# keichi/sdn-mpi-router

Hardware: AMD Instinct MI355X
Metric: all-pairs routes/sec + % HBM roofline, k=48 fat-tree, 1/2/4/8 MI355X (higher is better)
Workload: dtype int32; 1 GPU; fat_tree:48 all-pairs dfs route tables (find_route); fabric=fat_tree:48, V=2880, E=110592, table_layout=packed, endpoints=host-bearing switches (host pairs), parallelism=sources sharded over 1 GPU(s), steps_in_flight=1

## Files before the change

### sdn-mpi-router_amd/csrc/capi.hip

```cpp
#include <stdarg.h>
#include <stdio.h>
#include <stdlib.h>
#include <string.h>

#include <algorithm>
#include <array>
#include <map>
#include <string>
#include <thread>
#include <vector>

#include "common.h"

static thread_local char g_err[512] = "";

int sdnr_fail(int code, const char *fmt, ...)
{
    va_list ap;
    va_start(ap, fmt);
    vsnprintf(g_err, sizeof g_err, fmt, ap);
    va_end(ap);
    return code;
}

// ... 130 lines not shown
}

static void free_graph(sdnr_ctx *c)
{
    int32_t **bufs[] = {&c->row_ptr, &c->col, &c->port, &c->ell_col, &c->ell_port};
    for (int32_t **b : bufs) {
        if (*b) (void)hipFree(*b);
        *b = nullptr;
    }
    if (c->cost) (void)hipFree(c->cost);
    c->cost = nullptr;
    c->has_cost = false;
    if (c->twin_rep) (void)hipFree(c->twin_rep);
    c->twin_rep = nullptr;
    c->has_twins = false;
    ++c->upload_gen;
    memset(c->live_ring, 0, sizeof c->live_ring);
    if (c->radj16 && c->radj_owned) (void)hipFree(c->radj16);
    if (c->runs) (void)hipFree(c->runs);
    c->runs = nullptr;
    c->runs_R = 0;
    if (c->adjb) (void)hipFree(c->adjb);
    if (c->adjp) (void)hipFree(c->adjp);
    if (c->radjx) (void)hipFree(c->radjx);
    c->adjb = nullptr;
    c->adjp = nullptr;
    c->radjx = nullptr;
    if (c->q_radj16 && c->q_radj_owned) (void)hipFree(c->q_radj16);
    {
        void **qb[] = {reinterpret_cast<void **>(&c->q_adj16), reinterpret_cast<void **>(&c->q_deg32),
                       reinterpret_cast<void **>(&c->q_radjw), reinterpret_cast<void **>(&c->q_radjc),
                       reinterpret_cast<void **>(&c->q_cid), reinterpret_cast<void **>(&c->q_info),
                       reinterpret_cast<void **>(&c->q_loff), reinterpret_cast<void **>(&c->q_slot),
                       reinterpret_cast<void **>(&c->q_tab)};
        for (void **b : qb) {
            if (*b) (void)hipFree(*b);
            *b = nullptr;
        }
    }
    c->q_radj16 = nullptr;
    c->q_radj_owned = false;
    c->q_V = c->q_E = 0;
    if (c->adj16) (void)hipFree(c->adj16);
    if (c->deg32) (void)hipFree(c->deg32);
    if (c->radjw) (void)hipFree(c->radjw);
    c->radjw = nullptr;
    if (c->radjc) (void)hipFree(c->radjc);
    c->radjc = nullptr;
    if (c->dict_bp) (void)hipFree(c->dict_bp);
    if (c->dict_bt) (void)hipFree(c->dict_bt);
    if (c->dict_off) (void)hipFree(c->dict_off);
    c->dict_bp = nullptr;
    c->dict_bt = nullptr;
    c->dict_off = nullptr;
    c->dict_P = 0;
    c->dict_NB = 0;
    c->dict_bpw = 0;
    if (c->ell16) (void)hipFree(c->ell16);
    if (c->ell_hi) (void)hipFree(c->ell_hi);
    c->ell16 = nullptr;
    c->ell_hi = nullptr;
    c->adj16 = nullptr;
    c->radj16 = nullptr;
    c->deg32 = nullptr;
    c->radj_owned = false;
    c->radj_pair = false;
    c->V = -1;
// ... 591 lines not shown
            if (he == hipSuccess) he = hipMalloc(reinterpret_cast<void **>(&ctx->adjp), ap.size());
            if (he == hipSuccess)
                he = hipMemcpyAsync(ctx->adjp, ap.data(), ap.size(), hipMemcpyHostToDevice,
                                    ctx->stream);
            if (he == hipSuccess) he = hipMalloc(reinterpret_cast<void **>(&ctx->radjx), rx.size() * 4);
            if (he == hipSuccess)
                he = hipMemcpyAsync(ctx->radjx, rx.data(), rx.size() * 4, hipMemcpyHostToDevice,
                                    ctx->stream);
            if (he == hipSuccess) he = hipStreamSynchronize(ctx->stream);
        }
#endif
        if (he == hipSuccess) he = hipStreamSynchronize(ctx->stream);
        if (he != hipSuccess) {
            free_graph(ctx);
            return sdnr_hip_fail(he, "graph_upload(adj16)");
        }
        if (ctx->has_twins && ctx->radj16) {
            std::vector<int32_t> cmax_of((size_t)V), id_of((size_t)V, -1);
            for (int32_t v = 0; v < V; ++v) cmax_of[twin_rep[v]] = v;
            int32_t Vq = 0;
            for (int32_t v = 0; v < V; ++v)
                if (cmax_of[twin_rep[v]] == v) id_of[twin_rep[v]] = Vq++;
            std::vector<uint32_t> cidrk((size_t)V + kPad, 0u), info((size_t)Vq + 1, 0u),
                csize((size_t)Vq, 0u);
            for (int32_t v = 0; v < V; ++v) {
                const uint32_t c = (uint32_t)id_of[twin_rep[v]];
                cidrk[v] = c | (csize[c]++ << 16);
                info[c] = (uint32_t)v;
            }
            for (int32_t c = 0; c < Vq; ++c) info[c] |= csize[c] > 1 ? 1u << 16 : 0u;
            std::vector<int32_t> qptr((size_t)Vq + 1, 0), qcol, tmp;
            std::vector<uint32_t> loff((size_t)Vq * SDNR_WAVE + kPad, 0u);
            std::vector<uint8_t> mslot;
            for (int32_t c = 0; c < Vq; ++c) {
                const int32_t P = (int32_t)(info[c] & 0xFFFFu);
                tmp.clear();
                for (int32_t e = row_ptr[P]; e < row_ptr[P + 1]; ++e)
                    tmp.push_back((int32_t)(cidrk[col[e]] & 0xFFFFu));
                std::sort(tmp.begin(), tmp.end());
                tmp.erase(std::unique(tmp.begin(), tmp.end()), tmp.end());
                for (size_t j = 0; j < tmp.size(); ++j) {
                    loff[(size_t)c * SDNR_WAVE + j] = (uint32_t)mslot.size();
                    mslot.resize(mslot.size() + csize[tmp[j]], 0);
                }
                for (int32_t e = row_ptr[P]; e < row_ptr[P + 1]; ++e) {
                    const uint32_t ck = cidrk[col[e]];
                    const size_t j = (size_t)(std::lower_bound(tmp.begin(), tmp.end(),
                                                               (int32_t)(ck & 0xFFFFu)) - tmp.begin());
                    mslot[loff[(size_t)c * SDNR_WAVE + j] + (ck >> 16)] = (uint8_t)(e - row_ptr[P]);
                }
                qcol.insert(qcol.end(), tmp.begin(), tmp.end());
                qptr[(size_t)c + 1] = (int32_t)qcol.size();
            }
            mslot.resize(mslot.size() + kPad, 0);
            qcol.push_back(0);
            std::vector<uint16_t> qa16, qr16;
            bool qsym = true;
            int32_t qmaxin = 0;
            U16Rows q;
            he = upload_u16_rows(q, Vq, qptr.data(), qcol.data(), qa16, qr16, qsym, qmaxin,
                                 ctx->radj_pair ? 1 : 0);
            ctx->q_adj16 = q.adj16;
            ctx->q_radj16 = q.radj16;
            ctx->q_deg32 = q.deg32;
            ctx->q_radjw = q.radjw;
            ctx->q_radjc = q.radjc;
            ctx->q_radj_owned = q.radj_owned;
            auto put = [&](void **dst, const void *src, size_t bytes) {
                if (he == hipSuccess) he = hipMalloc(dst, bytes);
                if (he == hipSuccess)
                    he = hipMemcpyAsync(*dst, src, bytes, hipMemcpyHostToDevice, ctx->stream);
            };
            put(reinterpret_cast<void **>(&ctx->q_cid), cidrk.data(), cidrk.size() * 4);
            put(reinterpret_cast<void **>(&ctx->q_info), info.data(), info.size() * 4);
            put(reinterpret_cast<void **>(&ctx->q_loff), loff.data(), loff.size() * 4);
            put(reinterpret_cast<void **>(&ctx->q_slot), mslot.data(), mslot.size());
            const sdnr_quot qt{V, ctx->q_cid, ctx->q_info, ctx->q_loff, ctx->q_slot};
            put(reinterpret_cast<void **>(&ctx->q_tab), &qt, sizeof qt);
            if (he == hipSuccess) he = hipStreamSynchronize(ctx->stream);
            if (he != hipSuccess) {
                free_graph(ctx);
                return sdnr_hip_fail(he, "graph_upload(quotient)");
            }
            if (!ctx->radjw && ctx->q_radjw) {
                (void)hipFree(ctx->q_radjw);
                ctx->q_radjw = nullptr;
            }
            if (!ctx->radjc && ctx->q_radjc) {
                (void)hipFree(ctx->q_radjc);
                ctx->q_radjc = nullptr;
            }
            ctx->q_V = Vq;
            ctx->q_E = qptr[(size_t)Vq];
        }
    }
    bool symmetric = true;
    for (int32_t u = 0; u < V && symmetric; ++u)
        for (int32_t e = row_ptr[u]; e < row_ptr[u + 1]; ++e) {
            const int32_t v = col[e];
            int32_t lo = row_ptr[v], hi = row_ptr[v + 1];
            while (lo < hi) {
                const int32_t mid = (lo + hi) >> 1;
                if (col[mid] < u) lo = mid + 1; else hi = mid;
            }
            if (lo == row_ptr[v + 1] || col[lo] != u) {
                symmetric = false;
                break;
            }
        }
    SDNR_HIP(hipStreamSynchronize(ctx->stream));
// ... 1069 lines not shown
```

### sdn-mpi-router_amd/csrc/common.h

```cpp
#pragma once

#include <hip/hip_runtime.h>
#include <stdlib.h>
#include <stdint.h>
#include <stddef.h>

#include "../../include/sdnroute.h"

#define SDNR_WAVE 64
#define SDNR_LDS_PER_CU (160 * 1024)
#define SDNR_MAX_LDS_PER_BLOCK (160 * 1024)


__device__ __forceinline__ int lane_id() { return (int)__lane_id(); }

__device__ __forceinline__ int lanes_below(uint64_t m) {
    return (int)__builtin_amdgcn_mbcnt_hi((uint32_t)(m >> 32),
                                          __builtin_amdgcn_mbcnt_lo((uint32_t)m, 0u));
}

__device__ __forceinline__ int uniform(int x) {
    return __builtin_amdgcn_readfirstlane(x);
}

__device__ __forceinline__ int read_lane(int x, int lane) {
    return __builtin_amdgcn_readlane(x, lane);
}

__device__ __forceinline__ int highest_lane(uint64_t m) { return 63 - __clzll(m); }

__device__ __forceinline__ int lds_swz(int x) { return x ^ ((x >> 3) & 31); }


constexpr int kLiveRing = 8;

struct sdnr_quot {
    int32_t VR;
    const uint32_t *cid, *info, *loff;
    const uint8_t *slot;
};

struct sdnr_ctx {
    int device = 0;
    int num_cus = 256;
    hipStream_t own_stream = nullptr;
    hipStream_t stream = nullptr;

    int32_t V = -1, E = 0, max_deg = 0;
    uint64_t deg2_sum = 0;
    int32_t max_indeg = 0x7FFFFFFF;
    int32_t W = 0;
    int32_t *row_ptr = nullptr, *col = nullptr, *port = nullptr;
    uint32_t *cost = nullptr;
    bool has_cost = false;
    int32_t *ell_col = nullptr, *ell_port = nullptr;
    uint16_t *ell16 = nullptr;
    uint32_t *ell_hi = nullptr;
    uint32_t *dict_bp = nullptr;
    uint32_t *dict_bt = nullptr;
    int32_t *dict_off = nullptr;
    int32_t dict_P = 0, dict_NB = 0, dict_bpw = 0;
    uint16_t *adj16 = nullptr;
    uint16_t *radj16 = nullptr;
    uint32_t *deg32 = nullptr;
    uint16_t *radjw = nullptr;
    uint16_t *radjc = nullptr;
    bool radj_owned = false;
    bool radj_pair = false;
    uint32_t *runs = nullptr;
    int32_t runs_R = 0;
    uint64_t *adjb = nullptr;
    uint8_t *adjp = nullptr;
    uint32_t *radjx = nullptr;
    int32_t *twin_rep = nullptr;
    bool has_twins = false;
    int32_t q_V = 0, q_E = 0;
    uint16_t *q_adj16 = nullptr, *q_radj16 = nullptr, *q_radjw = nullptr, *q_radjc = nullptr;
    uint32_t *q_deg32 = nullptr;
    bool q_radj_owned = false;
    uint32_t *q_cid = nullptr, *q_info = nullptr, *q_loff = nullptr;
    uint8_t *q_slot = nullptr;
    struct sdnr_quot *q_tab = nullptr;
    bool dfs_quotient = false;
    int32_t dfs_nsrc = 0;
    bool dfs_folded = false;
    int32_t dfs_form = 0;
    unsigned long long *h_live = nullptr;
    struct {
        uint32_t seq0, seq1, gen;
        int32_t nsrc;
    } live_ring[kLiveRing] = {};
    int live_head = 0;
    uint32_t live_seq = 0;
    uint32_t upload_gen = 0;

    void *scratch = nullptr;
    size_t scratch_bytes = 0;
    void *stage = nullptr;
    size_t stage_bytes = 0;
    void *scratch2 = nullptr;
    size_t scratch2_bytes = 0;
    void *scratch3 = nullptr;
    size_t scratch3_bytes = 0;
    void *wq = nullptr;
    size_t wq_bytes = 0;
    void *dmat = nullptr;
    size_t dmat_bytes = 0;
    void *anc = nullptr;
    size_t anc_bytes = 0;
    const void *anc_parent = nullptr, *anc_port = nullptr;
    size_t anc_n = 0;
    bool anc_valid = false;
    bool port16 = false;
    bool symmetric = false;
// ... 190 lines not shown
```

### sdn-mpi-router_amd/csrc/dfs.hip

```cpp
#include <stdlib.h>
#include <string.h>

#include <type_traits>

#include "common.h"

namespace {

constexpr int kRing = 1024;

template <bool ELL, bool HOPS>
__global__ __launch_bounds__(64) void dfs_lds_wide_kernel(
    int V, int W, const int32_t *__restrict__ row_ptr,
    const int32_t *__restrict__ col, const int32_t *__restrict__ port,
    const int32_t *__restrict__ src, int nsrc, int32_t *__restrict__ out_parent,
    int32_t *__restrict__ out_port, int32_t *__restrict__ out_hops)
{
    extern __shared__ __attribute__((aligned(16))) uint32_t lds[];
    const int VW = (V + 31) >> 5;
    const int VWp = (VW + 3) & ~3;
    uint32_t *vis = lds;
    uint32_t *stk = vis + VWp;
    uint32_t *ps = stk + V;
    uint16_t *dep = reinterpret_cast<uint16_t *>(ps + V);
// ... 1402 lines not shown
            for (int v = lane; v < V; v += SDNR_WAVE) {
                if (((vis[vsw(v >> 5)] >> (v & 31)) & 1u) == 0u) {
                    prow[v] = -1;
                    if (!PACKED) trow[v] = -1;
                    if (HOPS) put_hop(out_hops, hb + v, -1, flags);
                }
            }
        }
        __builtin_amdgcn_fence(__ATOMIC_RELEASE, "workgroup", "local");
        if (lane == 0) __hip_atomic_store(&ctl[2 * NS + w], -1, __ATOMIC_RELAXED,
                                          __HIP_MEMORY_SCOPE_WORKGROUP);
#ifdef SDNR_STAMPS
        SDNR_STAMP(z_t1);
        if (lane == 0) {
            atomicAdd(&g_stamp[0], z_t1 - z_t0);
            atomicAdd(&g_stamp[1], z_rd);
            atomicAdd(&g_stamp[2], z_it);
            atomicAdd(&g_stamp[3], z_nl);
            atomicAdd(&g_stamp[4], z_qw);
            atomicAdd(&g_stamp[5], z_push);
            atomicAdd(&g_stamp[6], z_sp);
            atomicAdd(&g_stamp[7], z_rf);
            atomicAdd(&g_stamp[8], z_rfc);
        }
#endif
    } else {
        split_writer<NS, HOPS, PK>(V, W, ell_port, qrec, qdep, ctl, lane, out_parent, out_port,
                                   out_hops, err, flags);
    }
}

__device__ __forceinline__ int swz(int x) { return lds_swz(x); }

template <int NW, bool HOPS, bool PACKED, bool C16, int PAIR, bool SPEC = false, bool QUOT = false>
__global__ __launch_bounds__(NW * 64, C16 ? 7 : 1) void dfs_async_kernel(
    int V, const uint16_t *__restrict__ adj, const uint16_t *__restrict__ radj,
    const uint32_t *__restrict__ deg, const int32_t *__restrict__ row_ptr,
    const int32_t *__restrict__ port, int W, const int32_t *__restrict__ ell_port,
    const int32_t *__restrict__ src, int nsrc, int32_t *__restrict__ out_parent,
    int32_t *__restrict__ out_port, int32_t *__restrict__ out_hops, int *__restrict__ err,
    int flags, const int32_t *__restrict__ live,
    const sdnr_quot *__restrict__ qt)
{
    static_assert(NW >= 2, "wave 0 searches, the others decrement");
    constexpr bool quot = QUOT;
    const int VT = quot ? uniform((int)qt->VR) : V;
    if (live) nsrc = min(nsrc, *live);
    constexpr int U = 4;
    constexpr int S = NW - 1;
    constexpr int RING = 512;
#ifndef SDNR_ASYNC_G
#define SDNR_ASYNC_G 8
#endif
#ifndef SDNR_ASYNC_FLUSH_U
#define SDNR_ASYNC_FLUSH_U 6
#endif
#ifndef SDNR_ASYNC_G_DW
#define SDNR_ASYNC_G_DW 16
#endif
#ifndef SDNR_ASYNC_G_P1
#define SDNR_ASYNC_G_P1 8
#endif
#ifndef SDNR_ASYNC_G_U16
#define SDNR_ASYNC_G_U16 48
#endif
#ifndef SDNR_ASYNC_G_DW4
#define SDNR_ASYNC_G_DW4 32
#endif
    constexpr int G = NW <= 4 ? (PAIR == 0 ? SDNR_ASYNC_G_U16
                                           : (PAIR == 2 && NW == 4 ? SDNR_ASYNC_G_DW4 : SDNR_ASYNC_G))
                              : (PAIR == 2 ? SDNR_ASYNC_G_DW : (PAIR == 1 ? SDNR_ASYNC_G_P1 : 8));
    constexpr unsigned kSpin = 1u << 22;
    extern __shared__ __attribute__((aligned(16))) uint32_t lds[];
    const int VW = (V + 1 + 31) >> 5;
    const int VWp = (VW + 3) & ~3;
    const int CWp = ((((C16 ? (V + 2) >> 1 : V + 1) + 31) & ~31) + 64 + 255) & ~255;
    const int SWp = (((V + 1) >> 1) + 3) & ~3;
    const int PW = (V + 255) & ~255;
    const int PWp = C16 ? PW / 2 + PW / 4 : PW;
    uint32_t *vis = lds;
    uint32_t *cnt = vis + VWp;
    uint16_t *stk = reinterpret_cast<uint16_t *>(cnt + CWp);
    uint32_t *ps = cnt + CWp + SWp;
    uint16_t *ps16 = reinterpret_cast<uint16_t *>(ps);
    uint8_t *sl8 = reinterpret_cast<uint8_t *>(ps16 + PW);
    uint16_t *dep = reinterpret_cast<uint16_t *>(ps + PWp);
    auto cnt_of = [&](int v) -> uint32_t {
        if constexpr (C16) {
            const uint32_t x = __hip_atomic_load(&cnt[swz(v >> 1)], __ATOMIC_RELAXED,
                                                 __HIP_MEMORY_SCOPE_WORKGROUP);
            return (x >> ((v & 1) << 4)) & 0xFFFFu;
        } else {
            return __hip_atomic_load(&cnt[swz(v)], __ATOMIC_RELAXED, __HIP_MEMORY_SCOPE_WORKGROUP);
        }
    };
    uint16_t *ring = reinterpret_cast<uint16_t *>(ps + PWp + (HOPS ? ((V + 1) >> 1) : 0));
    int *ctl = reinterpret_cast<int *>(ring + RING);
    const int lane = lane_id();
    const int w = uniform((int)(threadIdx.x >> 6));
#ifdef SDNR_STAMPS
    unsigned long long kstart;
    SDNR_STAMP(kstart);
#endif

    for (int si = blockIdx.x; si < nsrc; si += gridDim.x) {
        const int sr = uniform(src[si]);
        int32_t *prow = out_parent + (size_t)si * VT;
        int32_t *trow = PACKED ? nullptr : out_port + (size_t)si * VT;
        const size_t hb = (size_t)si * VT;
        if (sr < 0 || sr >= VT) {
            for (int v = threadIdx.x; v < VT; v += blockDim.x) {
                prow[v] = -1;
                if (!PACKED) trow[v] = -1;
                if (HOPS) put_hop(out_hops, hb + v, -1, flags);
            }
            continue;
        }
        int s = sr;
        bool rootvis = true;
        if constexpr (quot) {
            s = uniform((int)(qt->cid[sr] & 0xFFFFu));
            rootvis = uniform((int)(qt->info[s] >> 16)) == 0;
        }
#ifdef SDNR_STAMPS
        unsigned long long ph0, ph1, ph2, ph3;
        SDNR_STAMP(ph0);
#endif
        for (int i = threadIdx.x; i < VW; i += blockDim.x) vis[i] = 0u;
        if constexpr (C16) {
            const int nw = (V + 2) >> 1;
            for (int i0 = threadIdx.x; i0 < nw; i0 += U * blockDim.x) {
                uint2 dg[U];
#pragma unroll
                for (int k = 0; k < U; ++k) {
                    const int i = i0 + k * (int)blockDim.x;
                    dg[k] = reinterpret_cast<const uint2 *>(deg)[i < nw ? i : 0];
                }
#pragma unroll
                for (int k = 0; k < U; ++k) {
                    const int i = i0 + k * (int)blockDim.x;
                    if (i < nw) cnt[swz(i)] = dg[k].x | (dg[k].y << 16);
                }
            }
        } else {
            for (int i0 = threadIdx.x; i0 <= V; i0 += U * blockDim.x) {
                uint32_t dg[U];
#pragma unroll
                for (int k = 0; k < U; ++k) {
                    const int i = i0 + k * (int)blockDim.x;
                    dg[k] = deg[i <= V ? i : V];
                }
#pragma unroll
                for (int k = 0; k < U; ++k) {
                    const int i = i0 + k * (int)blockDim.x;
                    if (i <= V) cnt[swz(i)] = dg[k];
                }
            }
        }
        if (threadIdx.x < 2 + S) ctl[threadIdx.x] = 0;
        __syncthreads();
#ifdef SDNR_STAMPS
        SDNR_STAMP(ph1);
#endif

        if (w == 0) {
            if (flags & kFlagPrio) __builtin_amdgcn_s_setprio(3);
            const int pub0 = rootvis ? 1 : 0;
            if (lane == 0) {
                if (rootvis) vis[s >> 5] |= 1u << (s & 31);
                vis[V >> 5] |= 1u << (V & 31);
                if (C16) ps16[swz(s)] = (uint16_t)s;
                else ps[swz(s)] = (uint32_t)s;
                if (HOPS) dep[s] = 0;
                stk[0] = (uint16_t)s;
                ring[0] = (uint16_t)s;
            }
            __builtin_amdgcn_fence(__ATOMIC_RELEASE, "workgroup");
            if (lane == 0) __hip_atomic_store(&ctl[0], pub0, __ATOMIC_RELAXED, __HIP_MEMORY_SCOPE_WORKGROUP);
            int pub = pub0, pubd = pub0, sp = 1, lo = 0;
            constexpr int NPF = 1;
            int pu[NPF];
            uint16_t xp[NPF];
#pragma unroll
            for (int k = 0; k < NPF; ++k) {
                pu[k] = -1;
                xp[k] = (uint16_t)V;
            }
#ifdef SDNR_STAMPS
            unsigned long long st_t0, st_t1, st_row = 0, st_cand = 0, st_false = 0, st_bp = 0,
                                               st_miss = 0, st_skip = 0, st_tc = 0, st_skipc = 0,
                                               st_pushc = 0;
            SDNR_STAMP(st_t0);
// ... 127 lines not shown
                    m = __ballot(c != 0u);
                    if (m) break;
                    sp -= kk;
                }
                if (pub != pubd) {
                    __builtin_amdgcn_fence(__ATOMIC_RELEASE, "workgroup", "local");
                    if (lane == 0) __hip_atomic_store(&ctl[0], pub, __ATOMIC_RELAXED,
                                                      __HIP_MEMORY_SCOPE_WORKGROUP);
                    pubd = pub;
                }
                if (!m) break;
                const int first = __ffsll((unsigned long long)m) - 1;
                sp -= first + 1;
                for (int u = read_lane(e, first); u >= 0;) u = explore(u);
            }
            __builtin_amdgcn_fence(__ATOMIC_RELEASE, "workgroup");
            if (lane == 0) __hip_atomic_store(&ctl[1], 1, __ATOMIC_RELAXED, __HIP_MEMORY_SCOPE_WORKGROUP);
            if (flags & kFlagPrio) __builtin_amdgcn_s_setprio(0);
#ifdef SDNR_STAMPS
            SDNR_STAMP(st_t1);
            if (lane == 0) {
                atomicAdd(&g_stamp[0], st_t1 - st_t0);
                atomicAdd(&g_stamp[1], st_row);
                atomicAdd(&g_stamp[2], st_cand);
                atomicAdd(&g_stamp[3], st_false);
                atomicAdd(&g_stamp[4], st_bp);
                atomicAdd(&g_stamp[5], st_skip * 1000000ull + st_miss);
                atomicAdd(&g_stamp[6], st_skipc);
                atomicAdd(&g_stamp[7], st_pushc);
            }
#endif
        } else {
            int j = w - 1;
            for (unsigned spin = 0;;) {
                const int P = __hip_atomic_load(&ctl[0], __ATOMIC_ACQUIRE, __HIP_MEMORY_SCOPE_WORKGROUP);
                if (j >= P) {
                    if (__hip_atomic_load(&ctl[1], __ATOMIC_ACQUIRE, __HIP_MEMORY_SCOPE_WORKGROUP) &&
                        j >= __hip_atomic_load(&ctl[0], __ATOMIC_ACQUIRE, __HIP_MEMORY_SCOPE_WORKGROUP))
                        break;
                    if (++spin > kSpin) {
                        if (lane == 0) atomicOr(err, 2);
                        break;
                    }
                    __builtin_amdgcn_s_sleep(1);
                    continue;
                }
                spin = 0;
                const int n = (P - j + S - 1) / S < G ? (P - j + S - 1) / S : G;
                const int mine = lane < n ? (int)ring[(j + lane * S) & (RING - 1)] : V;
                if constexpr (PAIR == 2) {
                    constexpr int G2 = G / 2;
                    const int hiw = lane >> 5;
                    const uint32_t *rw32 = reinterpret_cast<const uint32_t *>(radj);
                    uint32_t r[G2];
#pragma unroll
                    for (int g = 0; g < G2; ++g) {
                        const int ca = read_lane(mine, 2 * g), cb = read_lane(mine, 2 * g + 1);
                        r[g] = rw32[(size_t)(hiw ? cb : ca) * 32 + (lane & 31)];
                    }
#pragma unroll
                    for (int g = 0; g < G2; ++g)
                        if (2 * g + hiw < n) {
                            atomicSub(&cnt[r[g] & 0xFFFFu], 1u);
                            atomicSub(&cnt[r[g] >> 16], 1u);
                        }
                    j += n * S;
                    if (lane == 0) __hip_atomic_store(&ctl[2 + w - 1], j, __ATOMIC_RELAXED,
                                                      __HIP_MEMORY_SCOPE_WORKGROUP);
                    continue;
                }
                if constexpr (PAIR == 1) {
                    constexpr int G2 = G / 2;
                    const int hiw = lane >> 5;
                    int r[G2];
#pragma unroll
                    for (int g = 0; g < G2; ++g) {
                        const int ca = read_lane(mine, 2 * g), cb = read_lane(mine, 2 * g + 1);
                        r[g] = radj[(size_t)(hiw ? cb : ca) * 64 + lane];
                    }
#pragma unroll
                    for (int g = 0; g < G2; ++g)
                        if (2 * g + hiw < n) {
                            if (C16) atomicSub(&cnt[r[g] >> 1], 1u << ((r[g] & 1) << 4));
                            else atomicSub(&cnt[r[g]], 1u);
                        }
                    j += n * S;
                    if (lane == 0) __hip_atomic_store(&ctl[2 + w - 1], j, __ATOMIC_RELAXED,
                                                      __HIP_MEMORY_SCOPE_WORKGROUP);
                    continue;
                }
                int r[G];
#pragma unroll
                for (int g = 0; g < G; ++g) r[g] = radj[(size_t)read_lane(mine, g) * 64 + lane];
                if (flags & kFlagPreSwz) {
#pragma unroll
                    for (int g = 0; g < G; ++g)
                        if (g < n) {
                            if (C16) atomicSub(&cnt[r[g] >> 1], 1u << ((r[g] & 1) << 4));
                            else atomicSub(&cnt[r[g]], 1u);
                        }
                } else {
#pragma unroll
                    for (int g = 0; g < G; ++g)
                        if (g < n && r[g] != V) {
                            if (C16) atomicSub(&cnt[swz(r[g] >> 1)], 1u << ((r[g] & 1) << 4));
                            else atomicSub(&cnt[swz(r[g])], 1u);
                        }
                }
                j += n * S;
                if (lane == 0) __hip_atomic_store(&ctl[2 + w - 1], j, __ATOMIC_RELAXED, __HIP_MEMORY_SCOPE_WORKGROUP);
            }
        }
        __syncthreads();
#ifdef SDNR_STAMPS
        SDNR_STAMP(ph2);
#endif

        constexpr int UF = SDNR_ASYNC_FLUSH_U;
        if constexpr (quot) {
            const uint32_t *__restrict__ qcid = qt->cid, *__restrict__ qinfo = qt->info,
                                         *__restrict__ qloff = qt->loff;
            const uint8_t *__restrict__ qslot = qt->slot;
            for (int v0 = threadIdx.x; v0 < VT; v0 += UF * blockDim.x) {
                uint32_t ck[UF], lf[UF];
                int p[UF], sl[UF], pt[UF];
#pragma unroll
                for (int k = 0; k < UF; ++k) {
                    const int v = v0 + k * (int)blockDim.x;
                    ck[k] = qcid[v < VT ? v : 0];
                }
#pragma unroll
                for (int k = 0; k < UF; ++k) {
                    const int v = v0 + k * (int)blockDim.x;
                    const int c = (int)(ck[k] & 0xFFFFu);
                    p[k] = -1;
                    sl[k] = -1;
                    lf[k] = 0;
                    if (v < VT && v == sr) {
                        p[k] = sr;
                    } else if (v < VT && ((vis[c >> 5] >> (c & 31)) & 1u)) {
                        int pc, qs;
                        if (C16) {
                            pc = (int)ps16[swz(c)];
                            qs = (int)sl8[swz(c)];
                        } else {
                            const uint32_t xx = ps[swz(c)];
                            pc = (int)(xx & 0xFFFFu);
                            qs = (int)(xx >> 16);
                        }
                        p[k] = pc == s ? sr : (int)(qinfo[pc] & 0xFFFFu);
                        lf[k] = qloff[(size_t)pc * 64 + qs];
                        sl[k] = 0;
                    }
                }
#pragma unroll
                for (int k = 0; k < UF; ++k)
                    if (sl[k] >= 0) sl[k] = (int)qslot[lf[k] + (ck[k] >> 16)];
#pragma unroll
                for (int k = 0; k < UF; ++k) {
                    pt[k] = -1;
                    if (sl[k] >= 0)
                        pt[k] = W > 0 ? ell_port[(size_t)p[k] * W + sl[k]]
                                      : port[row_ptr[p[k]] + sl[k]];
                }
#pragma unroll
                for (int k = 0; k < UF; ++k) {
                    const int v = v0 + k * (int)blockDim.x;
                    if (v < VT) {
                        if (PACKED) {
                            prow[v] = (int32_t)(((uint32_t)p[k] & 0xFFFFu) |
                                                ((uint32_t)pt[k] << 16));
                        } else {
                            prow[v] = p[k];
                            trow[v] = pt[k];
                        }
                        if (HOPS)
                            put_hop(out_hops, hb + v,
                                    p[k] < 0 ? -1 : (v == sr ? 0 : (int)dep[ck[k] & 0xFFFFu]), flags);
                    }
                }
            }
        } else
        for (int v0 = threadIdx.x; v0 < V; v0 += UF * blockDim.x) {
            int p[UF], sl[UF], pt[UF];
#pragma unroll
            for (int k = 0; k < UF; ++k) {
                const int v = v0 + k * (int)blockDim.x;
                p[k] = -1;
                sl[k] = -1;
                if (v < V && ((vis[v >> 5] >> (v & 31)) & 1u)) {
                    if (C16) {
                        p[k] = (int)ps16[swz(v)];
                        if (v != s) sl[k] = (int)sl8[swz(v)];
                    } else {
                        const uint32_t xx = ps[swz(v)];
                        p[k] = (int)(xx & 0xFFFFu);
                        if (v != s) sl[k] = (int)(xx >> 16);
                    }
                }
            }
#pragma unroll
            for (int k = 0; k < UF; ++k) {
                pt[k] = -1;
                if (sl[k] >= 0)
                    pt[k] = W > 0 ? ell_port[(size_t)p[k] * W + sl[k]] : port[row_ptr[p[k]] + sl[k]];
            }
#pragma unroll
            for (int k = 0; k < UF; ++k) {
                const int v = v0 + k * (int)blockDim.x;
                if (v < V) {
                    if (PACKED) {
// ... 134 lines not shown
{
    if (K >= 16) launch_batch<ELL, HOPS, 16>(small, grid, lds, st, a);
    else if (K >= 8) launch_batch<ELL, HOPS, 8>(small, grid, lds, st, a);
    else if (K >= 4) launch_batch<ELL, HOPS, 4>(small, grid, lds, st, a);
    else launch_batch<ELL, HOPS, 1>(small, grid, lds, st, a);
}

template <bool HOPS>
void launch_wide(bool small, int grid, size_t lds, hipStream_t st, const DfsArgs &a)
{
    if (small) {
        auto k = dfs_lds_wide_kernel<false, HOPS>;
        allow_full_lds(k);
        hipLaunchKernelGGL(k, dim3(grid), dim3(64), lds, st, a.V, a.W, a.row_ptr, a.col, a.port,
                           a.src, a.nsrc, a.parent, a.port_out, a.hops);
    } else {
        auto k = dfs_global_wide_kernel<false, HOPS>;
        allow_full_lds(k);
        hipLaunchKernelGGL(k, dim3(grid), dim3(64), lds, st, a.V, a.W, a.row_ptr, a.col, a.port,
                           a.src, a.nsrc, a.parent, a.port_out, a.hops, a.spill);
    }
}

}

static size_t dfs_lds_bytes_count(int V, bool hops)
{
    const size_t VWp = (size_t)((((V + 1 + 31) >> 5) + 3) & ~3);
    const size_t CWp = (size_t)((V + 1 + 3) & ~3);
    const size_t SWp = (size_t)((((V + 1) >> 1) + 3) & ~3);
    return align16(4 * (VWp + CWp + SWp) + 4 * (size_t)V + (hops ? 2 * (size_t)V : 0));
}

static size_t dfs_lds_bytes_async(int V, bool hops, bool c16 = false)
{
    const size_t VWp = (size_t)((((V + 1 + 31) >> 5) + 3) & ~3);
    const size_t CWp = (size_t)(((((c16 ? (V + 2) >> 1 : V + 1) + 31) & ~31) + 64 + 255) & ~255);
    const size_t SWp = (size_t)((((V + 1) >> 1) + 3) & ~3);
    const size_t PW = (size_t)((V + 255) & ~255);
    const size_t PWp = c16 ? PW / 2 + PW / 4 : PW;
    return align16(4 * (VWp + CWp + SWp) + 4 * PWp +
                   (hops ? 4 * (size_t)((V + 1) >> 1) : 0) + 2 * 512 + 4 * 16);
}

static size_t dfs_lds_bytes_coop(int V)
{
    const size_t VWp = (size_t)((((V + 1 + 31) >> 5) + 3) & ~3);
    return align16(4 * VWp + 8 * (size_t)V + 4 * (size_t)((V + 1) >> 1) + 4 * 32);
}

namespace {

template <bool HOPS, int KW>
void launch_coop_kw(int grid, size_t lds, hipStream_t st, int V, const uint16_t *adj,
                    const DfsArgs &a)
{
    auto k = dfs_coop_kernel<4, KW, HOPS>;
    allow_full_lds(k);
    hipLaunchKernelGGL(k, dim3(grid), dim3(4 * 64), lds, st, V, adj, a.row_ptr,
                       a.port_csr, a.src, a.nsrc, a.parent, a.port_out,
                       a.hops);
}

template <bool HOPS>
void launch_coop(int kw, int grid, size_t lds, hipStream_t st, int V, const uint16_t *adj,
                 const DfsArgs &a)
{
    if (kw >= 8) launch_coop_kw<HOPS, 8>(grid, lds, st, V, adj, a);
    else if (kw >= 4) launch_coop_kw<HOPS, 4>(grid, lds, st, V, adj, a);
    else launch_coop_kw<HOPS, 2>(grid, lds, st, V, adj, a);
}

}

static int dfs_coop_kw()
// ... 258 lines not shown

static bool dfs_small(const sdnr_ctx *ctx, int nsrc)
{
    const int V = ctx->V;
    const size_t small_b = dfs_lds_bytes_small(V);
    const size_t cu_blocks_small = SDNR_LDS_PER_CU / small_b;
    bool small = V < 65536 && small_b <= 64 * 1024 &&
                 (small_b <= 40 * 1024 ||
                  (size_t)nsrc <= (size_t)ctx->num_cus * cu_blocks_small);
    if (const char *f = getenv("SDNROUTE_DFS_STRATEGY")) {
        if (!strcmp(f, "global")) small = false;
        else if ((!strcmp(f, "lds") || !strcmp(f, "coop") || !strcmp(f, "count") ||
                  !strcmp(f, "async")) && V < 65536 &&
                 small_b <= SDNR_MAX_LDS_PER_BLOCK)
            small = true;
    }
    return small;
}

static bool dfs_count_ok(const sdnr_ctx *ctx, bool hops)
{
    return ctx->adj16 != nullptr && ctx->radj16 != nullptr && ctx->V < 65535 &&
           dfs_lds_bytes_count(ctx->V, hops) <= SDNR_MAX_LDS_PER_BLOCK;
}

static bool dfs_async(const sdnr_ctx *ctx, int nsrc, bool hops)
{
    const char *force = getenv("SDNROUTE_DFS_STRATEGY");
    return dfs_count_ok(ctx, hops) &&
           dfs_lds_bytes_async(ctx->V, hops) <= SDNR_MAX_LDS_PER_BLOCK &&
           (force ? !strcmp(force, "async") : dfs_small(ctx, nsrc));
}

static bool dfs_quotient(const sdnr_ctx *ctx)
{
    if (!ctx->q_tab || ctx->q_V <= 0) return false;
    if (const char *f = getenv("SDNROUTE_DFS_QUOTIENT")) {
        if (!strcmp(f, "0")) return false;
        if (!strcmp(f, "1")) return true;
    }
    return 2 * (int64_t)ctx->q_E <= (int64_t)ctx->E;
}

#ifndef SDNR_FOLD_LOW_FORM
#define SDNR_FOLD_LOW_FORM 2
#endif

static int dfs_dispatch(sdnr_ctx *ctx, const int32_t *d_src, int32_t nsrc,
                        int32_t *d_parent, int32_t *d_port, int32_t *d_hops, uint32_t *d_tree,
                        bool slots = false, bool hops16 = false,
                        const int32_t *d_live = nullptr, bool low = false, int32_t live_n = 0)
{
    const int V = ctx->V;
    if (nsrc == 0 || V == 0) return SDNR_OK;
    const bool packed = d_tree != nullptr;
    const bool ell = ctx->W > 0;
    const bool hops = d_hops != nullptr;
    const bool narrow = ctx->max_deg <= SDNR_WAVE;
    const size_t small_b = dfs_lds_bytes_small(V);
    const bool small = dfs_small(ctx, nsrc);
    size_t lds = small ? small_b : dfs_lds_bytes_global(V);
    if (lds > SDNR_MAX_LDS_PER_BLOCK)
        return sdnr_fail(SDNR_ERR_INVAL, "graph too large for the LDS visited set (V=%d)", V);
    size_t bpc = SDNR_LDS_PER_CU / lds;
    if (bpc > 16) bpc = 16;
    if (bpc < 1) bpc = 1;
    int grid = (int)((size_t)ctx->num_cus * bpc);
    if (grid > nsrc) grid = nsrc;
    uint2 *spill = nullptr;
// ... 37 lines not shown
        int rc = sdnr_reserve(&ctx->scratch2, &ctx->scratch2_bytes,
                              (h16 ? 3 : 2) * n * sizeof(int32_t));
        if (rc) return rc;
        int32_t *tp = static_cast<int32_t *>(ctx->scratch2);
        int32_t *th = h16 ? tp + 2 * n : d_hops;
        if (!packed) {
            if ((rc = dfs_dispatch(ctx, d_src, nsrc, d_parent, d_port, tp, nullptr))) return rc;
            hipLaunchKernelGGL(dfs_hops16_kernel, dim3(ctx->num_cus * 8), dim3(256), 0,
                               ctx->stream, n, tp, reinterpret_cast<uint16_t *>(d_hops));
            SDNR_HIP(hipGetLastError());
            if (ctx->timed) SDNR_HIP(hipEventRecord(ctx->ev1, ctx->stream));
            return SDNR_OK;
        }
        if ((rc = dfs_dispatch(ctx, d_src, nsrc, tp, tp + n, th, nullptr))) return rc;
        if (h16)
            hipLaunchKernelGGL(dfs_hops16_kernel, dim3(ctx->num_cus * 8), dim3(256), 0,
                               ctx->stream, n, th, reinterpret_cast<uint16_t *>(d_hops));
        if (slots)
            hipLaunchKernelGGL(dfs_slot_pack_kernel, dim3(ctx->num_cus * 8), dim3(256), 0,
                               ctx->stream, n, V, tp, ctx->row_ptr, ctx->col, d_tree);
        else
            hipLaunchKernelGGL(dfs_pack_kernel, dim3(ctx->num_cus * 8), dim3(256), 0, ctx->stream,
                               n, tp, tp + n, d_tree);
        SDNR_HIP(hipGetLastError());
        if (ctx->timed) SDNR_HIP(hipEventRecord(ctx->ev1, ctx->stream));
        return SDNR_OK;
    }
    const bool count = !async && count_ok && (force ? !strcmp(force, "count") : small);
    const bool coop_ok = ctx->adj16 != nullptr && V < 65535 &&
                         dfs_lds_bytes_coop(V) <= SDNR_MAX_LDS_PER_BLOCK;
    const bool coop = !count && coop_ok && (force ? !strcmp(force, "coop") : small);
    if (async) {
        int *err = ctx->d_err;
        auto per_cu = [&](int w, bool c) {
            size_t b = SDNR_LDS_PER_CU / dfs_lds_bytes_async(V, hops, c);
            if (b > (size_t)(32 / w)) b = 32 / w;
            return b < 1 ? (size_t)1 : b;
        };
        auto compact = [&](int w) {
            bool c = per_cu(w, true) > per_cu(w, false) &&
                     (size_t)ctx->num_cus * per_cu(w, false) < (size_t)nsrc;
            if (const char *f = getenv("SDNROUTE_DFS_C16")) c = !strcmp(f, "1");
            return c;
        };
        const char *pz = getenv("SDNROUTE_DFS_PRESWZ");
        const bool quot = dfs_quotient(ctx);
        ctx->dfs_quotient = quot;
        auto rows_of = [&](bool c) {
            return quot ? (c ? ctx->q_radjc : ctx->q_radjw) : (c ? ctx->radjc : ctx->radjw);
        };
        auto preswz_of = [&](bool c) { return rows_of(c) && !(pz && !strcmp(pz, "0")); };
        int nw = dfs_async_waves(ctx, nsrc);
        if (low && d_live && live_n > 0) {
            const int cw = dfs_async_waves(ctx, live_n);
            const bool cc = compact(cw);
            if (!cc && !(preswz_of(cc) && ctx->radj_pair)) nw = cw;
        }
        const bool c16 = compact(nw);
        const size_t cl = dfs_lds_bytes_async(V, hops, c16);
        const size_t cpc = per_cu(nw, c16);
        const uint16_t *rw = rows_of(c16);
        const bool preswz = preswz_of(c16);
        bool specpop = true;
        if (const char *f = getenv("SDNROUTE_DFS_SPECPOP")) specpop = !strcmp(f, "1");
        bool spec = specpop;
        const int aflags = dfs_flags(kFlagPrio) | (preswz ? kFlagPreSwz : 0) | hflags |
                           (specpop ? kFlagSpecPop : 0);
        const bool pair = preswz && ctx->radj_pair;
        const char *dq = sdnr_tune_env("SDNROUTE_DFS_DW");
        bool dw = preswz && !pair && !c16 && nw >= 6;
        if (dq) dw = preswz && !pair && !c16 && !strcmp(dq, "1");
        if (low && d_live && !c16 && !pair) {
            if (SDNR_FOLD_LOW_FORM & 1) spec = false;
            if (SDNR_FOLD_LOW_FORM & 2) dw = preswz;
            ctx->dfs_form = kDfsFormLow;
        }
        int cgrid = (int)((size_t)ctx->num_cus * cpc);
        if (cgrid > nsrc) cgrid = nsrc;
        static const char *names[] = {"", "", "dfs_async_kernel<2>", "dfs_async_kernel<3>",
                                      "dfs_async_kernel<4>", "dfs_async_kernel<5>",
                                      "dfs_async_kernel<6>", "", "dfs_async_kernel<8>"};
        ctx->last_kernel = names[nw];
#define SDNR_ASYNC_P(N_, H_, P_)                                                             \
    do {                                                                                     \
        constexpr bool kSpecOk = N_ == 4;                    \
        auto k = quot ? (spec && kSpecOk ? async_pick<N_, H_, P_, kSpecOk, true>(c16, pair, dw) \
                                         : async_pick<N_, H_, P_, false, true>(c16, pair, dw)) \
                      : (spec && kSpecOk ? async_pick<N_, H_, P_, kSpecOk>(c16, pair, dw)    \
                                         : async_pick<N_, H_, P_, false>(c16, pair, dw));    \
        allow_full_lds(k);                                                                   \
        hipLaunchKernelGGL(k, dim3(cgrid), dim3(N_ * 64), cl, ctx->stream,                   \
                           quot ? ctx->q_V : V, quot ? ctx->q_adj16 : ctx->adj16,            \
// ... 624 lines not shown
```

Baseline: 14660 billion routes/s.

## Precompute quotient port table and record per-node slot offsets during DFS for flush

```diff
diff --git a/sdn-mpi-router_amd/csrc/capi.hip b/sdn-mpi-router_amd/csrc/capi.hip
--- a/sdn-mpi-router_amd/csrc/capi.hip
+++ b/sdn-mpi-router_amd/csrc/capi.hip
@@ -186,7 +186,7 @@
                        reinterpret_cast<void **>(&c->q_radjw), reinterpret_cast<void **>(&c->q_radjc),
                        reinterpret_cast<void **>(&c->q_cid), reinterpret_cast<void **>(&c->q_info),
                        reinterpret_cast<void **>(&c->q_loff), reinterpret_cast<void **>(&c->q_slot),
-                       reinterpret_cast<void **>(&c->q_tab)};
+                       reinterpret_cast<void **>(&c->q_port), reinterpret_cast<void **>(&c->q_tab)};
         for (void **b : qb) {
             if (*b) (void)hipFree(*b);
             *b = nullptr;
@@ -844,6 +844,7 @@
             std::vector<int32_t> qptr((size_t)Vq + 1, 0), qcol, tmp;
             std::vector<uint32_t> loff((size_t)Vq * SDNR_WAVE + kPad, 0u);
             std::vector<uint8_t> mslot;
+            std::vector<int32_t> mport;
             for (int32_t c = 0; c < Vq; ++c) {
                 const int32_t P = (int32_t)(info[c] & 0xFFFFu);
                 tmp.clear();
@@ -854,17 +855,20 @@
                 for (size_t j = 0; j < tmp.size(); ++j) {
                     loff[(size_t)c * SDNR_WAVE + j] = (uint32_t)mslot.size();
                     mslot.resize(mslot.size() + csize[tmp[j]], 0);
+                    mport.resize(mslot.size(), -1);
                 }
                 for (int32_t e = row_ptr[P]; e < row_ptr[P + 1]; ++e) {
                     const uint32_t ck = cidrk[col[e]];
                     const size_t j = (size_t)(std::lower_bound(tmp.begin(), tmp.end(),
                                                                (int32_t)(ck & 0xFFFFu)) - tmp.begin());
                     mslot[loff[(size_t)c * SDNR_WAVE + j] + (ck >> 16)] = (uint8_t)(e - row_ptr[P]);
+                    mport[loff[(size_t)c * SDNR_WAVE + j] + (ck >> 16)] = port[e];
                 }
                 qcol.insert(qcol.end(), tmp.begin(), tmp.end());
                 qptr[(size_t)c + 1] = (int32_t)qcol.size();
             }
             mslot.resize(mslot.size() + kPad, 0);
+            mport.resize(mslot.size(), -1);
             qcol.push_back(0);
             std::vector<uint16_t> qa16, qr16;
             bool qsym = true;
@@ -887,7 +891,8 @@
             put(reinterpret_cast<void **>(&ctx->q_info), info.data(), info.size() * 4);
             put(reinterpret_cast<void **>(&ctx->q_loff), loff.data(), loff.size() * 4);
             put(reinterpret_cast<void **>(&ctx->q_slot), mslot.data(), mslot.size());
-            const sdnr_quot qt{V, ctx->q_cid, ctx->q_info, ctx->q_loff, ctx->q_slot};
+            put(reinterpret_cast<void **>(&ctx->q_port), mport.data(), mport.size() * 4);
+            const sdnr_quot qt{V, ctx->q_cid, ctx->q_info, ctx->q_loff, ctx->q_slot, ctx->q_port};
             put(reinterpret_cast<void **>(&ctx->q_tab), &qt, sizeof qt);
             if (he == hipSuccess) he = hipStreamSynchronize(ctx->stream);
             if (he != hipSuccess) {
diff --git a/sdn-mpi-router_amd/csrc/common.h b/sdn-mpi-router_amd/csrc/common.h
--- a/sdn-mpi-router_amd/csrc/common.h
+++ b/sdn-mpi-router_amd/csrc/common.h
@@ -38,6 +38,7 @@
     int32_t VR;
     const uint32_t *cid, *info, *loff;
     const uint8_t *slot;
+    const int32_t *qport;
 };
 
 struct sdnr_ctx {
@@ -80,6 +81,7 @@
     bool q_radj_owned = false;
     uint32_t *q_cid = nullptr, *q_info = nullptr, *q_loff = nullptr;
     uint8_t *q_slot = nullptr;
+    int32_t *q_port = nullptr;
     struct sdnr_quot *q_tab = nullptr;
     bool dfs_quotient = false;
     int32_t dfs_nsrc = 0;
diff --git a/sdn-mpi-router_amd/csrc/dfs.hip b/sdn-mpi-router_amd/csrc/dfs.hip
--- a/sdn-mpi-router_amd/csrc/dfs.hip
+++ b/sdn-mpi-router_amd/csrc/dfs.hip
@@ -1458,6 +1458,13 @@
 
 __device__ __forceinline__ int swz(int x) { return lds_swz(x); }
 
+#ifndef SDNR_QUOT_FLUSH
+#define SDNR_QUOT_FLUSH 3
+#endif
+
+template <class T> using gptr = const __attribute__((address_space(1))) T *;
+template <class T> __device__ __forceinline__ gptr<T> as_global(const T *p) { return (gptr<T>)p; }
+
 template <int NW, bool HOPS, bool PACKED, bool C16, int PAIR, bool SPEC = false, bool QUOT = false>
 __global__ __launch_bounds__(NW * 64, C16 ? 7 : 1) void dfs_async_kernel(
     int V, const uint16_t *__restrict__ adj, const uint16_t *__restrict__ radj,
@@ -1522,6 +1529,9 @@
     };
     uint16_t *ring = reinterpret_cast<uint16_t *>(ps + PWp + (HOPS ? ((V + 1) >> 1) : 0));
     int *ctl = reinterpret_cast<int *>(ring + RING);
+    constexpr bool qf_port = quot && (SDNR_QUOT_FLUSH & 1), qf_rec = quot && (SDNR_QUOT_FLUSH & 2);
+    uint32_t *qlo = reinterpret_cast<uint32_t *>(ctl + 16);
+    int32_t *rport = reinterpret_cast<int32_t *>(qlo + ((V + 3) & ~3));
     const int lane = lane_id();
     const int w = uniform((int)(threadIdx.x >> 6));
 #ifdef SDNR_STAMPS
@@ -1552,6 +1562,11 @@
         unsigned long long ph0, ph1, ph2, ph3;
         SDNR_STAMP(ph0);
 #endif
+        int rp0 = -1;
+        if constexpr (qf_port) {
+            if (w == NW - 1)
+                rp0 = W > 0 ? ell_port[(size_t)sr * W + lane] : port[row_ptr[sr] + lane];
+        }
         for (int i = threadIdx.x; i < VW; i += blockDim.x) vis[i] = 0u;
         if constexpr (C16) {
             const int nw = (V + 2) >> 1;
@@ -1584,6 +1599,9 @@
             }
         }
         if (threadIdx.x < 2 + S) ctl[threadIdx.x] = 0;
+        if constexpr (qf_port) {
+            if (w == NW - 1) rport[lane] = rp0;
+        }
         __syncthreads();
 #ifdef SDNR_STAMPS
         SDNR_STAMP(ph1);
@@ -1777,6 +1795,8 @@
 #endif
         } else {
             int j = w - 1;
+            gptr<uint32_t> wloff = nullptr;
+            if constexpr (qf_rec) wloff = as_global(qt->loff);
             for (unsigned spin = 0;;) {
                 const int P = __hip_atomic_load(&ctl[0], __ATOMIC_ACQUIRE, __HIP_MEMORY_SCOPE_WORKGROUP);
                 if (j >= P) {
@@ -1793,6 +1813,17 @@
                 spin = 0;
                 const int n = (P - j + S - 1) / S < G ? (P - j + S - 1) / S : G;
                 const int mine = lane < n ? (int)ring[(j + lane * S) & (RING - 1)] : V;
+                uint32_t qo = 0u;
+                bool qrec = false;
+                if constexpr (qf_rec) {
+                    qrec = lane < n && (j + lane * S > 0 || !rootvis);
+                    if (qrec) {
+                        uint32_t xx;
+                        if (C16) xx = (uint32_t)ps16[swz(mine)] | ((uint32_t)sl8[swz(mine)] << 16);
+                        else xx = ps[swz(mine)];
+                        qo = wloff[(size_t)(xx & 0xFFFFu) * 64 + (xx >> 16)];
+                    }
+                }
                 if constexpr (PAIR == 2) {
                     constexpr int G2 = G / 2;
                     const int hiw = lane >> 5;
@@ -1809,6 +1840,9 @@
                             atomicSub(&cnt[r[g] & 0xFFFFu], 1u);
                             atomicSub(&cnt[r[g] >> 16], 1u);
                         }
+                    if constexpr (qf_rec) {
+                        if (qrec) qlo[mine] = qo;
+                    }
                     j += n * S;
                     if (lane == 0) __hip_atomic_store(&ctl[2 + w - 1], j, __ATOMIC_RELAXED,
                                                       __HIP_MEMORY_SCOPE_WORKGROUP);
@@ -1829,6 +1863,9 @@
                             if (C16) atomicSub(&cnt[r[g] >> 1], 1u << ((r[g] & 1) << 4));
                             else atomicSub(&cnt[r[g]], 1u);
                         }
+                    if constexpr (qf_rec) {
+                        if (qrec) qlo[mine] = qo;
+                    }
                     j += n * S;
                     if (lane == 0) __hip_atomic_store(&ctl[2 + w - 1], j, __ATOMIC_RELAXED,
                                                       __HIP_MEMORY_SCOPE_WORKGROUP);
@@ -1852,6 +1889,9 @@
                             else atomicSub(&cnt[swz(r[g])], 1u);
                         }
                 }
+                if constexpr (qf_rec) {
+                    if (qrec) qlo[mine] = qo;
+                }
                 j += n * S;
                 if (lane == 0) __hip_atomic_store(&ctl[2 + w - 1], j, __ATOMIC_RELAXED, __HIP_MEMORY_SCOPE_WORKGROUP);
             }
@@ -1863,12 +1903,14 @@
 
         constexpr int UF = SDNR_ASYNC_FLUSH_U;
         if constexpr (quot) {
-            const uint32_t *__restrict__ qcid = qt->cid, *__restrict__ qinfo = qt->info,
-                                         *__restrict__ qloff = qt->loff;
-            const uint8_t *__restrict__ qslot = qt->slot;
+            const gptr<uint32_t> qcid = as_global(qt->cid), qinfo = as_global(qt->info),
+                                 qloff = as_global(qt->loff);
+            const gptr<uint8_t> qslot = as_global(qt->slot);
+            const gptr<int32_t> qport = as_global(qt->qport);
             for (int v0 = threadIdx.x; v0 < VT; v0 += UF * blockDim.x) {
-                uint32_t ck[UF], lf[UF];
-                int p[UF], sl[UF], pt[UF];
+                uint32_t ck[UF], lf[UF], pi[UF], val[UF];
+                int p[UF], pt[UF], hp[UF];
+                bool ok[UF], rc[UF];
 #pragma unroll
                 for (int k = 0; k < UF; ++k) {
                     const int v = v0 + k * (int)blockDim.x;
@@ -1878,35 +1920,58 @@
                 for (int k = 0; k < UF; ++k) {
                     const int v = v0 + k * (int)blockDim.x;
                     const int c = (int)(ck[k] & 0xFFFFu);
-                    p[k] = -1;
-                    sl[k] = -1;
-                    lf[k] = 0;
-                    if (v < VT && v == sr) {
-                        p[k] = sr;
-                    } else if (v < VT && ((vis[c >> 5] >> (c & 31)) & 1u)) {
-                        int pc, qs;
-                        if (C16) {
-                            pc = (int)ps16[swz(c)];
-                            qs = (int)sl8[swz(c)];
-                        } else {
-                            const uint32_t xx = ps[swz(c)];
-                            pc = (int)(xx & 0xFFFFu);
-                            qs = (int)(xx >> 16);
-                        }
-                        p[k] = pc == s ? sr : (int)(qinfo[pc] & 0xFFFFu);
-                        lf[k] = qloff[(size_t)pc * 64 + qs];
-                        sl[k] = 0;
+                    const uint32_t vw = vis[c >> 5];
+                    uint32_t xx;
+                    if (C16) xx = (uint32_t)ps16[swz(c)] | ((uint32_t)sl8[swz(c)] << 16);
+                    else xx = ps[swz(c)];
+                    uint32_t off = 0u;
+                    if (qf_rec) off = qlo[c];
+                    int d = 0;
+                    if (HOPS) d = (int)dep[c];
+                    ok[k] = v < VT && v != sr && ((vw >> (c & 31)) & 1u);
+                    const int pc = ok[k] ? (int)(xx & 0xFFFFu) : 0;
+                    rc[k] = ok[k] && pc == s;
+                    p[k] = pc;
+                    if (qf_rec) lf[k] = ok[k] ? off + (ck[k] >> 16) : 0u;
+                    else lf[k] = ok[k] ? (uint32_t)pc * 64u + (xx >> 16) : 0u;
+                    hp[k] = ok[k] ? d : (v == sr ? 0 : -1);
+                }
+                if constexpr (!qf_rec) {
+#pragma unroll
+                    for (int k = 0; k < UF; ++k) pi[k] = qinfo[p[k]];
+#pragma unroll
+                    for (int k = 0; k < UF; ++k) {
+                        const uint32_t o = qloff[lf[k]];
+                        lf[k] = ok[k] ? o + (ck[k] >> 16) : 0u;
                     }
                 }
 #pragma unroll
-                for (int k = 0; k < UF; ++k)
-                    if (sl[k] >= 0) sl[k] = (int)qslot[lf[k] + (ck[k] >> 16)];
-#pragma unroll
                 for (int k = 0; k < UF; ++k) {
-                    pt[k] = -1;
-                    if (sl[k] >= 0)
-                        pt[k] = W > 0 ? ell_port[(size_t)p[k] * W + sl[k]]
-                                      : port[row_ptr[p[k]] + sl[k]];
+                    if (qf_rec) pi[k] = qinfo[p[k]];
+                    if (qf_port) {
+                        const gptr<uint32_t> at =
+                            rc[k] ? reinterpret_cast<gptr<uint32_t>>(qslot + (lf[k] & ~3u))
+                                  : reinterpret_cast<gptr<uint32_t>>(qport + lf[k]);
+                        val[k] = *at;
+                    } else {
+                        val[k] = (uint32_t)qslot[lf[k]];
+                    }
+                }
+#pragma unroll
+                for (int k = 0; k < UF; ++k) __asm__ volatile("" : "+v"(pi[k]), "+v"(val[k]));
+#pragma unroll
+                for (int k = 0; k < UF; ++k) {
+                    const int v = v0 + k * (int)blockDim.x;
+                    p[k] = ok[k] ? (rc[k] ? sr : (int)(pi[k] & 0xFFFFu)) : (v == sr ? sr : -1);
+                    if (qf_port) {
+                        const int own = rport[(val[k] >> ((lf[k] & 3u) << 3)) & 63u];
+                        pt[k] = ok[k] ? (rc[k] ? own : (int)val[k]) : -1;
+                    } else {
+                        const int pp = ok[k] ? p[k] : 0;
+                        pt[k] = W > 0 ? ell_port[(size_t)pp * W + val[k]]
+                                      : port[row_ptr[pp] + (int)val[k]];
+                        pt[k] = ok[k] ? pt[k] : -1;
+                    }
                 }
 #pragma unroll
                 for (int k = 0; k < UF; ++k) {
@@ -1919,9 +1984,7 @@
                             prow[v] = p[k];
                             trow[v] = pt[k];
                         }
-                        if (HOPS)
-                            put_hop(out_hops, hb + v,
-                                    p[k] < 0 ? -1 : (v == sr ? 0 : (int)dep[ck[k] & 0xFFFFu]), flags);
+                        if (HOPS) put_hop(out_hops, hb + v, hp[k], flags);
                     }
                 }
             }
@@ -2122,7 +2185,7 @@
     return align16(4 * (VWp + CWp + SWp) + 4 * (size_t)V + (hops ? 2 * (size_t)V : 0));
 }
 
-static size_t dfs_lds_bytes_async(int V, bool hops, bool c16 = false)
+static size_t dfs_lds_bytes_async(int V, bool hops, bool c16 = false, bool quot = false)
 {
     const size_t VWp = (size_t)((((V + 1 + 31) >> 5) + 3) & ~3);
     const size_t CWp = (size_t)(((((c16 ? (V + 2) >> 1 : V + 1) + 31) & ~31) + 64 + 255) & ~255);
@@ -2130,7 +2193,15 @@
     const size_t PW = (size_t)((V + 255) & ~255);
     const size_t PWp = c16 ? PW / 2 + PW / 4 : PW;
     return align16(4 * (VWp + CWp + SWp) + 4 * PWp +
-                   (hops ? 4 * (size_t)((V + 1) >> 1) : 0) + 2 * 512 + 4 * 16);
+                   (hops ? 4 * (size_t)((V + 1) >> 1) : 0) + 2 * 512 + 4 * 16 +
+                   (quot && (SDNR_QUOT_FLUSH & 3) ? 4 * (size_t)((V + 3) & ~3) + 4 * SDNR_WAVE : 0));
+}
+
+static size_t dfs_async_reserve(const sdnr_ctx *ctx, bool hops, bool c16, bool quot)
+{
+    const size_t g = dfs_lds_bytes_async(ctx->V, hops, c16);
+    const size_t q = quot ? dfs_lds_bytes_async(ctx->q_V, hops, c16, true) : 0;
+    return q > g ? q : g;
 }
 
 static size_t dfs_lds_bytes_coop(int V)
@@ -2455,9 +2526,10 @@
            (force ? !strcmp(force, "async") : dfs_small(ctx, nsrc));
 }
 
-static bool dfs_quotient(const sdnr_ctx *ctx)
+static bool dfs_quotient(const sdnr_ctx *ctx, bool hops)
 {
     if (!ctx->q_tab || ctx->q_V <= 0) return false;
+    if (dfs_async_reserve(ctx, hops, false, true) > SDNR_MAX_LDS_PER_BLOCK) return false;
     if (const char *f = getenv("SDNROUTE_DFS_QUOTIENT")) {
         if (!strcmp(f, "0")) return false;
         if (!strcmp(f, "1")) return true;
@@ -2561,8 +2633,10 @@
     const bool coop = !count && coop_ok && (force ? !strcmp(force, "coop") : small);
     if (async) {
         int *err = ctx->d_err;
+        const bool quot = dfs_quotient(ctx, hops);
+        ctx->dfs_quotient = quot;
         auto per_cu = [&](int w, bool c) {
-            size_t b = SDNR_LDS_PER_CU / dfs_lds_bytes_async(V, hops, c);
+            size_t b = SDNR_LDS_PER_CU / dfs_async_reserve(ctx, hops, c, quot);
             if (b > (size_t)(32 / w)) b = 32 / w;
             return b < 1 ? (size_t)1 : b;
         };
@@ -2573,8 +2647,6 @@
             return c;
         };
         const char *pz = getenv("SDNROUTE_DFS_PRESWZ");
-        const bool quot = dfs_quotient(ctx);
-        ctx->dfs_quotient = quot;
         auto rows_of = [&](bool c) {
             return quot ? (c ? ctx->q_radjc : ctx->q_radjw) : (c ? ctx->radjc : ctx->radjw);
         };
@@ -2586,7 +2658,7 @@
             if (!cc && !(preswz_of(cc) && ctx->radj_pair)) nw = cw;
         }
         const bool c16 = compact(nw);
-        const size_t cl = dfs_lds_bytes_async(V, hops, c16);
+        const size_t cl = dfs_async_reserve(ctx, hops, c16, quot);
         const size_t cpc = per_cu(nw, c16);
         const uint16_t *rw = rows_of(c16);
         const bool preswz = preswz_of(c16);
```

New measurement: 15120 billion routes/s, median of 6. +3.1%, better.
